# antbern/gridmap-slam-robot

Hardware: AMD Instinct MI355X
Metric: particle-scan evals/sec (higher is better)
Workload: dtype f64; 1 GPU; C3: 16384 particles/GPU x 720 beams (697 hits), 2048x2048 grid @ 0.02 m, full scan step (score+normalise+resample+ray-cast+likelihood rebuild; the rebuild is dirty-tile / factor-table-only: bit-identical results, likelihoodData on demand -- the reference's own every-cell rebuild is cpu_baseline.gpu_like_for_like_ms_per_step); particles_total=16384, particles_per_gpu=16384, beams=720, maps=1, maps_total=1, parallelism=single GPU, inputs=resident in HBM

## Files before the change

### gridmap_slam_robot_amd/csrc/gms_fused_kernels.hip

```cpp
#include "gms_map_kernels.hip"
#include "gms_pf_kernels.hip"
#include "gms_slam_kernels.hip"

#ifndef GMS_APPLY_BLOCKS_RIDING
#define GMS_APPLY_BLOCKS_RIDING 512
#endif

#ifndef RCF_RAYS
#define RCF_RAYS 4
#endif

template <bool LOGNORM>
__global__ void __launch_bounds__(256)
k_norm_raycast(GridDev g, const gms_beam *__restrict__ beams, int32_t B, uint32_t *__restrict__ cnt, int32_t *__restrict__ bbox,
               int32_t nw_max, uint32_t n_ray_blocks,
               const double *__restrict__ partials, int64_t nblk_global, double *__restrict__ w, const float *__restrict__ pose,
               int32_t n, int64_t offset, PackedParticle *__restrict__ packed, double *__restrict__ cum,
               double *__restrict__ chunk_tot, int64_t nchunks, double *__restrict__ p2, PfStatsDev *__restrict__ stats,
               uint32_t n_norm_blocks, double *__restrict__ logd, uint32_t *__restrict__ cnt_pend, const int32_t *__restrict__ bbox_pend,
               uint32_t n_near_blocks, const double *__restrict__ logw_lognorm, uint32_t *__restrict__ res_ticket,
               double *__restrict__ res_pre) {
    extern __shared__ __align__(16) unsigned char smem[];
    GMS_STAMP(GMS_STAMP_ROW(2, blockIdx.x), 0);
    if (blockIdx.x >= n_ray_blocks + n_norm_blocks) {
        apply_body(g, logd, cnt_pend, bbox_pend, nullptr, blockIdx.x - n_ray_blocks - n_norm_blocks, 0,
                   gridDim.x - n_ray_blocks - n_norm_blocks);
        GMS_STAMP(GMS_STAMP_ROW(2, blockIdx.x), 15);
        return;
    }
    if (blockIdx.x < n_ray_blocks) {
        __shared__ RedLds L;
        __shared__ float s_pose[3];
        const int cols[4] = { COL_SUM, COL_XW, COL_YW, COL_TW };
        double f[4];
        if (LOGNORM) {
            fold_lognorm<4>(partials, nblk_global, cols, f, L);
// ... 1 lines not shown
            fold_sums<4>(partials, nblk_global, cols, f, L);
        }
        if (threadIdx.x == 0) {
            s_pose[0] = (float)(f[1] / f[0]);
            s_pose[1] = (float)(f[2] / f[0]);
            s_pose[2] = (float)(f[3] / f[0]);
        }
        __syncthreads();
        GMS_STAMP(GMS_STAMP_ROW(2, blockIdx.x), 1);
        if (blockIdx.x >= n_ray_blocks - n_near_blocks)
            raycast_near_body(g, beams, B, B, nullptr, 0, cnt, bbox, blockIdx.x - (n_ray_blocks - n_near_blocks), 0, smem, s_pose);
        else
            raycast_body<false, RCF_RAYS, 4>(g, beams, B, B, nullptr, 0, nullptr, cnt, bbox, nullptr, nullptr, 0, nullptr, nw_max, blockIdx.x, 0,
                                             smem, s_pose, n_near_blocks ? 1 : 0);
    } else {
        normalize_pack_body(partials, nblk_global, w, pose, n, offset, packed, cum, chunk_tot, nchunks, p2, stats,
                            blockIdx.x - n_ray_blocks, 0, LOGNORM ? logw_lognorm : (const double *)nullptr, res_ticket, n_norm_blocks,
                            res_pre, smem);
        GMS_STAMP(GMS_STAMP_ROW(2, blockIdx.x), 14);
    }
}

__global__ void __launch_bounds__(256)
k_partials_apply(double *__restrict__ w, double *__restrict__ logw, const float *__restrict__ pose, int32_t n, int64_t offset,
                 int64_t nblk_global, double *__restrict__ partials, const double *__restrict__ part, int32_t part_nseg,
                 GridDev g, double *__restrict__ logd, uint32_t *__restrict__ cnt, const int32_t *__restrict__ bbox,
                 int32_t *__restrict__ bbox_idle, PfStatsDev *__restrict__ lognorm_stats) {
    if (blockIdx.x < (uint32_t)nblk_global)
        partials_body(w, logw, pose, n, offset, nblk_global, partials, part, part_nseg, blockIdx.x, blockIdx.y, lognorm_stats);
    else
        apply_body(g, logd, cnt, bbox, bbox_idle, blockIdx.x - (uint32_t)nblk_global, blockIdx.y, gridDim.x - (uint32_t)nblk_global);
}

// ... 78 lines not shown
                double d_center, double d_theta, gms_beam *__restrict__ beams_out, uint32_t n_deskew_blocks,
                float *__restrict__ pose, float *__restrict__ cs, int32_t n, int64_t offset, double d_center_sd, double d_theta_sd,
                uint64_t seed, uint64_t sequence) {
    if (blockIdx.x < n_deskew_blocks)
        deskew_body(angle, distance, hit, length, d_center, d_theta, beams_out, (int32_t)(blockIdx.x * 256u + threadIdx.x));
    else
        motion_body(pose, cs, n, offset, d_center, d_theta, d_center_sd, d_theta_sd, seed, sequence, 0,
                    (int32_t)((blockIdx.x - n_deskew_blocks) * 256u + threadIdx.x));
}

bool gms_can_pair_launches(const gms_pf *pf, int32_t B) {
    const gms_map *m = pf->map;
    return pf->n_maps == 1 && B > 0 && B <= GMS_MAX_BEAMS && !m->need_full_build && m->pair_launches;
}

void gms_launch_norm_raycast(gms_pf *pf, const double *d_partials, PackedParticle *d_packed_local, bool own,
                             const gms_beam *d_beams, int32_t B) {
    gms_map *m = pf->map;
    ProfScope ps(m, GMS_K_RAYCAST);
    const uint32_t n_near = rc_near_blocks(m, B);
    const uint32_t n_ray = (uint32_t)((B + RCF_RAYS - 1) / RCF_RAYS) + n_near, n_norm = (uint32_t)((pf->n + 255) / 256);
    const int64_t nch = nchunks_of(pf);
    const size_t smem_pre = own ? (size_t)(nch + 1 + (nch + 63) / 64 + 1) * sizeof(double) : 0;
    size_t smem = rc_smem(m, RCF_RAYS, n_near);
    if (smem < smem_pre) smem = smem_pre;
    uint32_t n_apply = 0;
    if (m->apply_pending) {
        const int32_t all = ((m->gd.W + APPLY_TW - 1) / APPLY_TW) * ((m->gd.H + APPLY_TH - 1) / APPLY_TH);
        n_apply = (uint32_t)(all < GMS_APPLY_BLOCKS_RIDING ? all : GMS_APPLY_BLOCKS_RIDING);
    }
    int32_t *pend = m->d_bbox + (size_t)m->bbox_cur * 4;
    int32_t *bb = n_apply ? m->d_bbox + (size_t)(1 - m->bbox_cur) * 4 : pend;
    const bool lognorm = gms_pf_lognorm_now(pf);
#define NR_LAUNCH(LN)                                                                                                                 \
    do {                                                                                                                              \
        if (smem > 48 * 1024)                                                                                                         \
            hipFuncSetAttribute(reinterpret_cast<const void *>(&k_norm_raycast<LN>), hipFuncAttributeMaxDynamicSharedMemorySize, (int)smem); \
        hipLaunchKernelGGL(k_norm_raycast<LN>, dim3(n_ray + n_norm + n_apply), dim3(256), smem, m->stream, m->gd, d_beams, B, m->d_cnt, bb, \
                           rc_nw_max(m), n_ray, d_partials, nblk_global_of(pf), pf->d_w, pf->d_pose, pf->n, pf->offset, d_packed_local, \
                           own ? pf->d_cum : (double *)nullptr, own ? pf->d_chunk_tot : (double *)nullptr, nchunks_of(pf),          \
                           own ? pf->d_p2 : (double *)nullptr, pf->d_stats, n_norm, m->d_log, m->d_cnt_pend, pend, n_near,          \
                           LN ? (const double *)pf->d_logw : (const double *)nullptr, own ? pf->d_res_ticket : (uint32_t *)nullptr,       \
                           pf->d_res_pre);                                                                                              \
    } while (0)
    if (lognorm) NR_LAUNCH(true); else NR_LAUNCH(false);
#undef NR_LAUNCH
    if (n_apply) gms_apply_done(m);
    pf_normalized(pf, own, own);
}

void gms_launch_partials_apply(gms_pf *pf, double *d_partials, bool apply_rides_later) {
    gms_map *m = pf->map;
    if (!m->apply_pending || apply_rides_later) { gms_launch_pf_partials(pf, d_partials); return; }
    ProfScope ps(m, GMS_K_REDUCE);
    const int64_t nblk = nblk_global_of(pf);
    const int32_t all = ((m->gd.W + APPLY_TW - 1) / APPLY_TW) * ((m->gd.H + APPLY_TH - 1) / APPLY_TH);
    const uint32_t n_apply = (uint32_t)(all < GMS_APPLY_BLOCKS ? all : GMS_APPLY_BLOCKS);
    int32_t *cur = m->d_bbox + (size_t)m->bbox_cur * m->n_maps * 4, *idle = m->d_bbox + (size_t)(1 - m->bbox_cur) * m->n_maps * 4;
    PfStatsDev *lognorm_stats = gms_pf_lognorm_now(pf) ? pf->d_stats : (PfStatsDev *)nullptr;
    hipLaunchKernelGGL(k_partials_apply, dim3((uint32_t)nblk + n_apply, pf->n_maps), dim3(256), 0, m->stream, pf->d_w, pf->d_logw,
                       pf->d_pose, pf->n, pf->offset, nblk, d_partials,
                       pf->pending_nseg ? (const double *)pf->d_part : (const double *)nullptr, pf->pending_nseg, m->gd, m->d_log,
                       m->d_cnt_pend, cur, idle, lognorm_stats);
    pf_weights_combined(pf);
    gms_apply_done(m);
}

void gms_launch_lik_resample(gms_pf *pf, double fraction) {
// ... 92 lines not shown
```

### gridmap_slam_robot_amd/csrc/gms_host.hip

```cpp
#include <math.h>
#include <dlfcn.h>
#include <stdarg.h>
#include <stddef.h>
#include <stdio.h>
#include <stdlib.h>
#include <string.h>

#include <new>
#include <algorithm>
#include <vector>

#include "gms_internal.h"

static thread_local char g_err[512] = "";

int gms_fail(int code, const char *fmt, ...) {
    va_list ap;
    va_start(ap, fmt);
    vsnprintf(g_err, sizeof(g_err), fmt, ap);
    va_end(ap);
    return code;
}

static int32_t j_d2i_host(double d) {
// ... 1277 lines not shown
    return slam_update_impl(pf, nullptr, &mo, dev_beams, B, B, r01, resample_fraction, integrate);
}

static int slam_update_impl(gms_pf *pf, const float *dev_xytheta, const MotionModel *motion, const gms_beam *dev_beams, int32_t B,
                            int32_t beam_stride, const double *r01, double resample_fraction, int32_t integrate) {
    REQUIRE(pf && dev_beams && r01, "null argument");
    int rc = refuse_owned_maps(pf);
    if (rc) return rc;
    gms_map *m = pf->map;
    if (pf_is_shard(pf))
        return gms_fail(GMS_ERR_STATE, "sharded filter: the collectives belong to the caller (see distributed.py)");
    const ScanIn at_pose = dev_scan(dev_beams, B, beam_stride, nullptr, pf, 0);
    rc = set_poses_and_score_dev(pf, dev_xytheta, dev_beams, B, beam_stride, pf->refine != 0, motion);
    const bool pair = !rc && integrate && !pf->reference_order && beam_stride == B;
    if (pair && gms_can_pair_launches(pf, B)) {
        gms_launch_partials_apply(pf, pf->d_partials, true);
        gms_launch_norm_raycast(pf, pf->d_partials, pf->d_global_own, true, dev_beams, B);
        return paired_likelihood_resample(pf, r01, resample_fraction);
    }
    if (pair && pf->n_maps > 1 && B > 0 && !m->need_full_build && m->pair_launches) {
        const bool ride = gms_raycast_tiled(m, B);
        gms_launch_partials_apply(pf, pf->d_partials, ride);
        gms_launch_pf_apply_partials(pf, pf->d_partials, pf->d_global_own, true);
        ScanDev d;
        scan_pose(m, at_pose, &d);
        gms_launch_raycast(m, dev_beams, B, B, d.poses, d.pose_stride, ride);
        return paired_likelihood_resample(pf, r01, resample_fraction);
    }
    if (!rc) rc = gms_pf_normalize(pf, nullptr);
    if (!rc && resample_fraction >= 0.0) rc = gms_pf_resample_if(pf, r01, resample_fraction);
    if (!rc && integrate) rc = map_scan(m, at_pose, SCAN_UPDATE_MAY_DEFER);
    return rc;
// ... 517 lines not shown
```

### gridmap_slam_robot_amd/csrc/gms_internal.h

```cpp
#pragma once

#include <hip/hip_runtime.h>
#include <stdint.h>

#include <vector>

#include "gridmapslam.h"

struct GridDev {
    int32_t W, H;
    int64_t cells;
    double posx, posy;
    double res;
    double rinv;
    float resf;
    double l_free, l_occ;
    int32_t extra;
    float half_tol;
    double z_hit;
    double c_rand;
    double inv_max;
    int32_t ktaps, khalf;
    int32_t fpitch;
    uint32_t fneutral;
// ... 359 lines not shown
bool gms_set_stamp_buffer(gms_map *m, void *dev_buffer);
void gms_launch_spin(gms_map *m, double us);
void gms_launch_copy(gms_map *m, void *dst, const void *src, size_t nbytes);
void gms_invalidate_tile_state(gms_map *m);
void gms_launch_get_raw(gms_map *m, int32_t mi, int32_t x, int32_t y, double *d_out2);
void gms_launch_debug_f32(gms_map *m, int32_t op, const float *d_a, float *d_out, int64_t n);
int gms_view_check(const gms_view *v, int32_t W, int32_t H, const char *what, int64_t *bytes);
int gms_view_staging(gms_map *m, int64_t image_bytes, unsigned char **base);
void gms_launch_view(gms_map *m, const double *src, const gms_view *v, void *d_out);

void gms_launch_pf_init(gms_pf *pf);
void gms_launch_pf_pose_trig(gms_pf *pf, const float *d_src);
void gms_launch_pf_combine(gms_pf *pf);
void gms_launch_pf_motion(gms_pf *pf, double d_center, double d_theta, uint64_t seed, uint64_t sequence);
void gms_launch_pf_chunk_sums(gms_pf *pf);
void gms_launch_partials_apply(gms_pf *pf, double *d_partials, bool apply_rides_later = false);
bool gms_can_pair_launches(const gms_pf *pf, int32_t B);
void gms_launch_norm_raycast(gms_pf *pf, const double *d_partials, PackedParticle *d_packed_local, bool own,
                             const gms_beam *d_beams, int32_t B);
void gms_launch_lik_resample(gms_pf *pf, double fraction);
void gms_launch_deskew_motion(gms_pf *pf, const double *d_angle, const double *d_distance, const uint8_t *d_hit, int32_t length,
                              double d_center, double d_theta, uint64_t seed, uint64_t sequence);
void gms_launch_partials_pack_apply(gms_pf *pf, bool apply_rides_later = false);
void gms_launch_raycast_norm_chunks(gms_pf *pf, const gms_beam *d_beams, int32_t B, bool raycast);
void gms_launch_pf_fold_neff(gms_pf *pf);
struct MotionModel {
    double d_center, d_theta;
    uint64_t seed, sequence;
};
static inline void motion_deviations(double d_center, double d_theta, double *d_center_sd, double *d_theta_sd) {
    *d_center_sd = (0.01 + fabs(d_center) * 0.05) / 2;
    *d_theta_sd = 5 * (3.141592653589793 / 180.0) + 0.1 * fabs(d_theta);
}
void gms_launch_pf_score(gms_pf *pf, const gms_beam *d_beams, int32_t B, int32_t beam_stride, const float *d_pose_src = nullptr,
                         const MotionModel *motion = nullptr);
void gms_launch_pf_partials(gms_pf *pf, double *d_partials);
bool gms_pf_lognorm_now(const gms_pf *pf);
void gms_launch_pf_pack(gms_pf *pf, PackedParticle *d_packed);
void gms_launch_pf_apply_partials(gms_pf *pf, const double *d_partials, PackedParticle *d_packed_local, bool own);
void gms_launch_pf_stats_only(gms_pf *pf, const double *d_partials, PfStatsDev *d_stats_out);
void gms_launch_pf_resample(gms_pf *pf, double fraction );
void gms_launch_pf_refine(gms_pf *pf, const gms_beam *d_beams, int32_t B, int32_t beam_stride);
void gms_launch_pf_normalize_seq(gms_pf *pf, PfStatsDev *d_stats_out, bool normalise);
void gms_launch_pf_resample_seq(gms_pf *pf, double fraction);
SlamBufs gms_slam_bufs(const gms_slam *s);
void gms_launch_slam_likelihood(gms_map *m, const SlamBufs &sb, int32_t n);
void gms_launch_slam_deskew(gms_map *m, const double *angle, const double *distance, const uint8_t *hit, int32_t L, int32_t S, int32_t Lmax,
                            int32_t length, double d_center, double d_theta, const SlamFilterArgs *tab_src, SlamFilterArgs *tab_dst, gms_beam *d_out,
                            int32_t out_pitch);
void gms_launch_slam_particle(gms_pf *pf, const gms_beam *d_beams, int32_t B, const SlamBufs &sb, bool field_in_memory, const MotionModel *motion,
                              int32_t integrate, int64_t code_words, const SlamBatch *batch = nullptr);
void gms_launch_slam_likelihood_codes(gms_map *m, const SlamBufs &sb, int64_t code_words, int32_t n, int32_t plane);
// ... 33 lines not shown
```

### gridmap_slam_robot_amd/csrc/gms_pf_kernels.hip

```cpp
#include "gms_device.h"

#define SCAN_CHUNK 64
#define RES_SUB_MAX_CHUNKS 1024

__global__ void k_pf_init(float *pose, float *cs, double *w, double *logw, int64_t total, double w0) {
    int64_t i = (int64_t)blockIdx.x * blockDim.x + threadIdx.x;
    if (i < total) {
        pose[3 * i] = 0.0f; pose[3 * i + 1] = 0.0f; pose[3 * i + 2] = 0.0f;
        cs[2 * i] = 1.0f; cs[2 * i + 1] = 0.0f;
        w[i] = w0; logw[i] = 0.0;
    }
}

__global__ void __launch_bounds__(256)
k_pose_trig(const float *__restrict__ src, float *__restrict__ dst, float *__restrict__ cs, int64_t total) {
    const int64_t i = (int64_t)blockIdx.x * blockDim.x + threadIdx.x;
    if (i >= total) return;
    const float x = src[3 * i], y = src[3 * i + 1], th = src[3 * i + 2];
    dst[3 * i] = x; dst[3 * i + 1] = y; dst[3 * i + 2] = th;
    float c, s;
    pose_trig(th, c, s);
    cs[2 * i] = c; cs[2 * i + 1] = s;
}

// ... 384 lines not shown
    double m[GMS_PARTIAL_STRIDE][MAX_WAVES];
};

#define COL_SUM 0
#define COL_MAX 1
#define COL_ARG 2
#define COL_NZ 3
#define COL_MLW 4
#define COL_SQ 5
#define COL_XW 6
#define COL_YW 7
#define COL_TW 8

static_assert(EPT == 1, "the log-normalising form of block_partials takes one particle per thread");
__device__ __forceinline__ double lognorm_ref(double m) { return m > -INFINITY ? m : 0.0; }
__device__ __forceinline__ void block_partials(double *__restrict__ w, double *__restrict__ logw,
                                               const float *__restrict__ pose, int64_t cnt, int64_t base,
                                               double out[GMS_PARTIAL_STRIDE], RedLds &L,
                                               const double *__restrict__ part = nullptr, int32_t part_mi = 0,
                                               int32_t part_n = 0, int32_t part_nseg = 0, int64_t part_p0 = 0,
                                               bool lognorm = false) {
    const int32_t tl = threadIdx.x & (GRP - 1);
    double s = 0.0, nz = 0.0, mv = -INFINITY, mx = 9.0e15, ml = -INFINITY, sq = 0.0, xw = 0.0, yw = 0.0, tw = 0.0;
#pragma unroll
    for (int e0 = 0; e0 < EPT; e0 += EPB) {
        double v[EPB], lw[EPB];
        float px[EPB], py[EPB], pt[EPB];
#pragma unroll
        for (int e = 0; e < EPB; e++) {
            const int64_t i = tl + (e0 + e) * GRP;
            const bool in = i < cnt;
            if (part) {
                v[e] = 0.0; lw[e] = -INFINITY;
                if (in) {
                    combine_segments(part, part_mi, part_n, part_nseg, part_p0 + i, v[e], lw[e]);
                    w[i] = v[e]; logw[i] = lw[e];
                }
            } else {
                v[e] = in ? w[i] : 0.0;
                lw[e] = in ? logw[i] : -INFINITY;
            }
            px[e] = in ? pose[3 * i] : 0.0f; py[e] = in ? pose[3 * i + 1] : 0.0f; pt[e] = in ? pose[3 * i + 2] : 0.0f;
        }
        if (lognorm) {
            double mloc = lw[0] == lw[0] ? lw[0] : -INFINITY;
#define GMS_STEP_(O) { const double v2 = wave_xor<O>(mloc); if (v2 > mloc) mloc = v2; }
            GMS_BUTTERFLY(GMS_STEP_)
#undef GMS_STEP_
            const int32_t wv = threadIdx.x >> 6, g4 = (wv >> 2) << 2;
            __syncthreads();
            if ((threadIdx.x & 63) == 0) L.b[wv] = mloc;
            __syncthreads();
            double mb = L.b[g4];
            for (int k = 1; k < 4; k++) if (L.b[g4 + k] > mb) mb = L.b[g4 + k];
            if (tl < cnt) v[0] = exp(lw[0] - lognorm_ref(mb));
        }
#pragma unroll
        for (int e = 0; e < EPB; e++) {
            const int64_t i = tl + (e0 + e) * GRP;
            if (i < cnt) {
                s += v[e];
                sq += v[e] * v[e];
                xw += (double)px[e] * v[e];
                yw += (double)py[e] * v[e];
                tw += angle_constrain((double)pt[e]) * v[e];
                if (v[e] == 0.0) nz += 1.0;
                const double key = lognorm ? lw[e] : v[e];
                if (key > mv) { mv = key; mx = (double)(base + i); }
                else if (mx > 8.0e15 && key == key) { mv = key; mx = (double)(base + i); }
                if (lw[e] > ml) ml = lw[e];
            }
        }
    }
    GMS_STAMP(GMS_STAMP_ROW(1, blockIdx.x), 2);
    double sums[6] = { s, nz, sq, xw, yw, tw };
#pragma unroll
    for (int c = 0; c < 6; c++) sums[c] = wave_sum_f64(sums[c]);
    double mli = 0.0;
#define GMS_STEP_(O) { const double v2 = wave_xor<O>(mv), i2 = wave_xor<O>(mx); argmax_merge(mv, mx, v2, i2); \
                       const double l2 = wave_xor<O>(ml); if (l2 > ml) ml = l2; }
    GMS_BUTTERFLY(GMS_STEP_)
#undef GMS_STEP_
    const int32_t wave = threadIdx.x >> 6, g4 = (wave >> 2) << 2;
    GMS_STAMP(GMS_STAMP_ROW(1, blockIdx.x), 3);
    __syncthreads();
    if ((threadIdx.x & 63) == 0) {
#pragma unroll
        for (int c = 0; c < 6; c++) L.m[c][wave] = sums[c];
        L.m[6][wave] = mv; L.m[7][wave] = mx; L.m[8][wave] = ml;
    }
    __syncthreads();
    GMS_STAMP(GMS_STAMP_ROW(1, blockIdx.x), 4);
#pragma unroll
    for (int c = 0; c < 6; c++) sums[c] = ((L.m[c][g4] + L.m[c][g4 + 1]) + L.m[c][g4 + 2]) + L.m[c][g4 + 3];
    mv = L.m[6][g4]; mx = L.m[7][g4]; ml = L.m[8][g4];
    for (int k = 1; k < 4; k++) {
        argmax_merge(mv, mx, L.m[6][g4 + k], L.m[7][g4 + k]);
        if (L.m[8][g4 + k] > ml) ml = L.m[8][g4 + k];
    }
    (void)mli;
    out[COL_SUM] = sums[0]; out[COL_NZ] = sums[1]; out[COL_SQ] = sums[2];
    out[COL_XW] = sums[3]; out[COL_YW] = sums[4]; out[COL_TW] = sums[5];
    out[COL_MAX] = mv; out[COL_ARG] = mx; out[COL_MLW] = ml;
}

__device__ __forceinline__ double fold_sum(const double *__restrict__ p, int64_t nblk, int col, double *lds) {
    double acc = 0.0;
    for (int64_t b = threadIdx.x & (GRP - 1); b < nblk; b += GRP) acc += p[b * GMS_PARTIAL_STRIDE + col];
    return group_sum(acc, lds);
}

template <int NC>
__device__ __forceinline__ void fold_sums(const double *__restrict__ p, int64_t nblk, const int (&col)[NC], double (&out)[NC],
                                          RedLds &L) {
    static_assert(NC <= GMS_PARTIAL_STRIDE, "RedLds::m has GMS_PARTIAL_STRIDE rows");
    double acc[NC];
#pragma unroll
// ... 86 lines not shown
    for (int c = 0; c < NC; c++) out[c] = ((L.m[c][g4] + L.m[c][g4 + 1]) + L.m[c][g4 + 2]) + L.m[c][g4 + 3];
    return M;
}

__device__ __forceinline__ void fold_argmax(const double *__restrict__ p, int64_t nblk, int colv, int coli, double &mv,
                                            double &mx, RedLds &L) {
    mv = -INFINITY; mx = 9.0e15;
    bool first = true;
    for (int64_t b = threadIdx.x & (GRP - 1); b < nblk; b += GRP) {
        const double v2 = p[b * GMS_PARTIAL_STRIDE + colv], i2 = coli >= 0 ? p[b * GMS_PARTIAL_STRIDE + coli] : (double)b;
        if (first) { mv = v2; mx = i2; first = false; } else argmax_merge(mv, mx, v2, i2);
    }
    group_argmax(mv, mx, L.a, L.b);
}

__device__ __forceinline__ double fold_stats(const double *__restrict__ p, int64_t nblk, PfStatsDev *s, bool write,
                                             const float *__restrict__ pose, int64_t pose_base, int64_t pose_n, RedLds &L,
                                             const PackedParticle *__restrict__ glob = nullptr, bool lognorm = false, double *ref_out = nullptr) {
    double ml = 0.0, mli;
    if (!write) {
        if (!lognorm) return fold_sum(p, nblk, COL_SUM, L.a);
        const int c1[1] = { COL_SUM };
        double f1[1];
        ml = fold_lognorm<1>(p, nblk, c1, f1, L);
        if (ref_out) *ref_out = ml;
        return f1[0];
    }
    const int cols[5] = { COL_SUM, COL_NZ, COL_XW, COL_YW, COL_TW };
    double f[5];
    if (lognorm) { ml = fold_lognorm<5>(p, nblk, cols, f, L); if (ref_out) *ref_out = ml; }
    else fold_sums<5>(p, nblk, cols, f, L);
    const double sum = f[0], nz = f[1], xw = f[2], yw = f[3], tw = f[4];
    double mv, mx;
    fold_argmax(p, nblk, COL_MAX, COL_ARG, mv, mx, L);
    if (!lognorm) fold_argmax(p, nblk, COL_MLW, -1, ml, mli, L);
    if (threadIdx.x == 0) {
        s->n_ambiguous = 0;
        s->weight_sum = sum;
        s->max_w = lognorm ? exp(ml - lognorm_ref(ml)) : mv;
        s->strongest = mx < 8.0e15 ? (int32_t)mx : 0;
        if (!lognorm) s->n_zero = (int32_t)nz;
// ... 25 lines not shown
    for (int64_t b = threadIdx.x & (GRP - 1); b < nblk; b += GRP) { a += load_coherent<COHERENT>(&p2[2 * b]); q += load_coherent<COHERENT>(&p2[2 * b + 1]); }
    norm_sum = group_sum(a, lds);
    const double qq = group_sum(q, lds);
    sq_sum = qq / (norm_sum * norm_sum);
}

__global__ void __launch_bounds__(256)
k_fold_neff(const double *__restrict__ p2_all, int64_t nblk, PfStatsDev *__restrict__ stats) {
    __shared__ RedLds L;
    const int32_t mi = blockIdx.x;
    double ns, sq;
    fold_neff(p2_all + (size_t)mi * nblk * 2, nblk, ns, sq, L.a);
    if (threadIdx.x == 0) { stats[mi].norm_sum = ns; stats[mi].sq_sum = sq; }
}

__device__ __forceinline__ void
partials_body(double *__restrict__ w, double *__restrict__ logw, const float *__restrict__ pose, int32_t n,
              int64_t offset, int64_t nblk_global, double *__restrict__ partials, const double *__restrict__ part,
              int32_t part_nseg, uint32_t bx, uint32_t by, PfStatsDev *__restrict__ lognorm_stats = nullptr) {
    __shared__ RedLds L;
    const int32_t mi = (int32_t)by;
    if (lognorm_stats && bx == 0 && threadIdx.x == 0) lognorm_stats[mi].n_zero = 0;
    const int64_t gb = bx;
    const int64_t lb = gb - offset / GMS_BLOCK;
    const int64_t nlb = ((int64_t)n + GMS_BLOCK - 1) / GMS_BLOCK;
    double *p = partials + ((size_t)mi * nblk_global + gb) * GMS_PARTIAL_STRIDE;
    if (lb < 0 || lb >= nlb) {
        if (threadIdx.x < GMS_PARTIAL_STRIDE) p[threadIdx.x] = 0.0;
        return;
    }
    double out[GMS_PARTIAL_STRIDE];
    const size_t o = (size_t)mi * n + lb * GMS_BLOCK;
    block_partials(w + o, logw + o, pose + 3 * o, block_count(n, lb), offset + lb * GMS_BLOCK, out, L, part, mi, n,
                   part_nseg, lb * GMS_BLOCK, lognorm_stats != nullptr);
    if (threadIdx.x == 0)
        for (int k = 0; k < GMS_PARTIAL_STRIDE; k++) p[k] = out[k];
}

__global__ void __launch_bounds__(256)
k_partials(double *__restrict__ w, double *__restrict__ logw, const float *__restrict__ pose, int32_t n,
           int64_t offset, int64_t nblk_global, double *__restrict__ partials, const double *__restrict__ part,
           int32_t part_nseg, PfStatsDev *__restrict__ lognorm_stats) {
    GMS_STAMP(GMS_STAMP_ROW(1, blockIdx.x), 0);
    partials_body(w, logw, pose, n, offset, nblk_global, partials, part, part_nseg, blockIdx.x, blockIdx.y, lognorm_stats);
    GMS_STAMP(GMS_STAMP_ROW(1, blockIdx.x), 1);
}

__device__ __forceinline__ double *chunk_sub_of(double *chunk_tot_all, int64_t nchunks, int32_t n_maps, int32_t mi) {
    return chunk_tot_all + (size_t)n_maps * (nchunks + 1) + (size_t)mi * nchunks * 8;
}
__device__ __forceinline__ void block_chunk_scan(double v, int64_t i, int64_t n_pop, int64_t blk, int64_t nchunks,
                                                 double *__restrict__ cum, double *__restrict__ chunk_tot,
                                                 double *__restrict__ p2_blk, double *__restrict__ sub, bool through = false) {
    __shared__ double s_ct[4][2];
    const int32_t lane = threadIdx.x & 63, wave = threadIdx.x >> 6;
    double inc = v;
#pragma unroll
    for (int o = 1; o < 64; o <<= 1) {
        const double up = __shfl_up(inc, o, GMS_WAVE);
// ... 48 lines not shown
                const double up = __shfl_up(inc, o, GMS_WAVE);
                if (lane >= o) inc += up;
            }
            const double excl = __shfl_up(inc, 1, GMS_WAVE);
            if (sidx < nsuper) sup[sidx] = s0 == 0 ? (lane == 0 ? 0.0 : excl) : carry + (lane == 0 ? 0.0 : excl);
            const double tot = __shfl(inc, 63, GMS_WAVE);
            carry = s0 == 0 ? tot : carry + tot;
        }
        if (lane == 0) off[nchunks] = carry;
    }
    __syncthreads();
    for (int64_t c = 64 + threadIdx.x; c < nchunks; c += blockDim.x) off[c] = sup[c >> 6] + off[c];
    __syncthreads();
}

__device__ __forceinline__ void
resample_prefix_last(const double *__restrict__ p2, int64_t nblk, const double *__restrict__ tot, int64_t nchunks, uint32_t *__restrict__ ticket,
                     uint32_t n_blocks, double *__restrict__ pre, PfStatsDev *__restrict__ stats, unsigned char *smem, double *lds) {
    __shared__ int32_t s_last;
    asm volatile("s_waitcnt vmcnt(0)" ::: "memory");
    __syncthreads();
    if (threadIdx.x == 0) {
        const uint32_t t = __hip_atomic_fetch_add(ticket, 1u, __ATOMIC_RELAXED, __HIP_MEMORY_SCOPE_AGENT);
        s_last = t == n_blocks - 1;
        if (s_last) __hip_atomic_store(ticket, 0u, __ATOMIC_RELAXED, __HIP_MEMORY_SCOPE_AGENT);
    }
    __syncthreads();
    if (!s_last) return;
    double *off = reinterpret_cast<double *>(smem);
    double tv[8];
#pragma unroll
    for (int k = 0; k < 8; k++) { const int64_t c = (int64_t)threadIdx.x + k * (int64_t)blockDim.x; tv[k] = c < nchunks ? load_coherent<true>(&tot[c]) : 0.0; }
    double norm_sum, sq_sum;
// ... 1 lines not shown
#pragma unroll
    for (int k = 0; k < 8; k++) { const int64_t c = (int64_t)threadIdx.x + k * (int64_t)blockDim.x; if (c < nchunks) off[c] = tv[k]; }
    for (int64_t c0 = (int64_t)threadIdx.x + 8 * (int64_t)blockDim.x; c0 < nchunks; c0 += 8 * (int64_t)blockDim.x) {
        double v[8];
#pragma unroll
        for (int k = 0; k < 8; k++) { const int64_t c = c0 + k * (int64_t)blockDim.x; v[k] = c < nchunks ? load_coherent<true>(&tot[c]) : 0.0; }
#pragma unroll
        for (int k = 0; k < 8; k++) { const int64_t c = c0 + k * (int64_t)blockDim.x; if (c < nchunks) off[c] = v[k]; }
    }
    chunk_offsets_scan(off, nchunks);
    for (int64_t c = threadIdx.x; c <= nchunks; c += blockDim.x) pre[c] = off[c];
    if (threadIdx.x == 0) {
        pre[nchunks + 1] = norm_sum; pre[nchunks + 2] = sq_sum;
        stats->norm_sum = norm_sum; stats->sq_sum = sq_sum;
    }
    GMS_STAMP(GMS_STAMP_ROW(2, blockIdx.x), 13);
}

__device__ __forceinline__ void
normalize_pack_body(const double *__restrict__ partials_all, int64_t nblk_global, double *__restrict__ w,
                    const float *__restrict__ pose, int32_t n, int64_t offset, PackedParticle *__restrict__ packed,
                    double *__restrict__ cum, double *__restrict__ chunk_tot, int64_t nchunks,
                    double *__restrict__ p2_all, PfStatsDev *__restrict__ stats, uint32_t bx, uint32_t by,
                    const double *__restrict__ logw_lognorm = nullptr, uint32_t *__restrict__ ticket = nullptr,
                    uint32_t n_blocks = 0, double *__restrict__ pre = nullptr, unsigned char *smem = nullptr) {
    __shared__ RedLds L;
    const int32_t mi = (int32_t)by;
    const double *p = partials_all + (size_t)mi * nblk_global * GMS_PARTIAL_STRIDE;
    double M = 0.0;
    const double sum = fold_stats(p, nblk_global, stats + mi, bx == 0, pose + (size_t)mi * n * 3, offset, n, L, nullptr, logw_lognorm != nullptr, &M);
    const int32_t i = (int32_t)bx * 256 + threadIdx.x;
    double wn = 0.0;
    if (logw_lognorm) {
        const double v = i < n ? exp(logw_lognorm[(size_t)mi * n + i] - lognorm_ref(M)) : 1.0;
        const int32_t zeros = __popcll(__ballot(v == 0.0));
        if ((threadIdx.x & 63) == 0 && zeros) atomicAdd(&stats[mi].n_zero, zeros);
        if (i < n) w[(size_t)mi * n + i] = v;
    }
    if (i < n) {
        const size_t gi = (size_t)mi * n + i;
        wn = w[gi] / sum;
        w[gi] = wn;
        PackedParticle pp;
        pp.w = wn; pp.x = pose[3 * gi]; pp.y = pose[3 * gi + 1]; pp.theta = pose[3 * gi + 2]; pp.pad = 0u;
        packed[gi] = pp;
    }
    if (cum)
        block_chunk_scan(wn, i, n, bx, nchunks, cum + (size_t)mi * n, chunk_tot + (size_t)mi * (nchunks + 1),
                         p2_all + ((size_t)mi * nblk_global + bx) * 2, chunk_sub_of(chunk_tot, nchunks, (int32_t)gridDim.y, mi),
                         ticket != nullptr);
    if (cum && ticket) resample_prefix_last(p2_all + (size_t)mi * nblk_global * 2, nblk_global, chunk_tot + (size_t)mi * (nchunks + 1),
                                            nchunks, ticket + mi, n_blocks, pre + (size_t)mi * (nchunks + 3), stats + mi, smem, L.a);
}

__global__ void __launch_bounds__(256)
k_normalize_pack(const double *__restrict__ partials_all, int64_t nblk_global, double *__restrict__ w,
                 const float *__restrict__ pose, int32_t n, int64_t offset, PackedParticle *__restrict__ packed,
                 double *__restrict__ cum, double *__restrict__ chunk_tot, int64_t nchunks,
                 double *__restrict__ p2_all, PfStatsDev *__restrict__ stats, const double *__restrict__ logw_lognorm) {
    normalize_pack_body(partials_all, nblk_global, w, pose, n, offset, packed, cum, chunk_tot, nchunks, p2_all, stats, blockIdx.x,
                        blockIdx.y, logw_lognorm);
}

__device__ __forceinline__ void
chunk_sums_body(const PackedParticle *__restrict__ glob_all, int64_t n_global, int64_t nchunks, double *__restrict__ cum_all,
                double *__restrict__ chunk_tot, double *__restrict__ p2_all, int64_t nblk_global, PfStatsDev *__restrict__ stats,
                uint32_t bx, uint32_t by) {
// ... 515 lines not shown
    if (motion) { std::swap(pf->d_pose, pf->d_pose2); std::swap(pf->d_cs, pf->d_cs2); }
    pf_scored(pf, nseg);
}

void gms_launch_pf_combine(gms_pf *pf) {
    if (!pf->pending_nseg) return;
    gms_map *m = pf->map;
    ProfScope ps(m, GMS_K_SCORE);
    hipLaunchKernelGGL(k_score_combine, dim3((pf->n + 255) / 256, pf->n_maps), dim3(256), 0, m->stream, pf->d_part, pf->n,
                       pf->pending_nseg, pf->d_w, pf->d_logw);
    pf_weights_combined(pf);
}

bool gms_pf_lognorm_now(const gms_pf *pf) { return pf->log_norm && pf->score_fresh; }

void gms_launch_pf_partials(gms_pf *pf, double *d_partials) {
    gms_map *m = pf->map;
    ProfScope ps(m, GMS_K_REDUCE);
    const int64_t nblk = nblk_global_of(pf);
    hipLaunchKernelGGL(k_partials, dim3((unsigned)nblk, pf->n_maps), dim3(256), 0, m->stream, pf->d_w, pf->d_logw,
                       pf->d_pose, pf->n, pf->offset, nblk, d_partials,
                       pf->pending_nseg ? (const double *)pf->d_part : (const double *)nullptr, pf->pending_nseg,
                       gms_pf_lognorm_now(pf) ? pf->d_stats : (PfStatsDev *)nullptr);
    pf_weights_combined(pf);
}

void gms_launch_pf_apply_partials(gms_pf *pf, const double *d_partials, PackedParticle *d_packed_local, bool own) {
    gms_map *m = pf->map;
    ProfScope ps(m, GMS_K_REDUCE);
    const int64_t nblk = nblk_global_of(pf);
    hipLaunchKernelGGL(k_normalize_pack, dim3((pf->n + 255) / 256, pf->n_maps), dim3(256), 0, m->stream, d_partials, nblk,
                       pf->d_w, pf->d_pose, pf->n, pf->offset, d_packed_local, own ? pf->d_cum : (double *)nullptr,
                       own ? pf->d_chunk_tot : (double *)nullptr, nchunks_of(pf), own ? pf->d_p2 : (double *)nullptr, pf->d_stats,
                       gms_pf_lognorm_now(pf) ? (const double *)pf->d_logw : (const double *)nullptr);
    pf_normalized(pf, own, false);
}

void gms_launch_pf_stats_only(gms_pf *pf, const double *d_partials, PfStatsDev *d_stats_out) {
// ... 73 lines not shown
```

Baseline: 371.0 million particle-scan evals/s.

## Defer argmax/zero/max-logw stats from partials kernel into normalise-pack pass

```diff
diff --git a/gridmap_slam_robot_amd/csrc/gms_fused_kernels.hip b/gridmap_slam_robot_amd/csrc/gms_fused_kernels.hip
--- a/gridmap_slam_robot_amd/csrc/gms_fused_kernels.hip
+++ b/gridmap_slam_robot_amd/csrc/gms_fused_kernels.hip
@@ -10,7 +10,7 @@
 #define RCF_RAYS 4
 #endif
 
-template <bool LOGNORM>
+template <bool LOGNORM, bool DEFER>
 __global__ void __launch_bounds__(256)
 k_norm_raycast(GridDev g, const gms_beam *__restrict__ beams, int32_t B, uint32_t *__restrict__ cnt, int32_t *__restrict__ bbox,
                int32_t nw_max, uint32_t n_ray_blocks,
@@ -18,8 +18,9 @@
                int32_t n, int64_t offset, PackedParticle *__restrict__ packed, double *__restrict__ cum,
                double *__restrict__ chunk_tot, int64_t nchunks, double *__restrict__ p2, PfStatsDev *__restrict__ stats,
                uint32_t n_norm_blocks, double *__restrict__ logd, uint32_t *__restrict__ cnt_pend, const int32_t *__restrict__ bbox_pend,
-               uint32_t n_near_blocks, const double *__restrict__ logw_lognorm, uint32_t *__restrict__ res_ticket,
-               double *__restrict__ res_pre) {
+               uint32_t n_near_blocks, const double *__restrict__ logw, uint32_t *__restrict__ res_ticket,
+               double *__restrict__ res_pre, double *partials_rw) {
+    static_assert(!(LOGNORM && DEFER), "the block-relative partial vector needs every column in front of this launch");
     extern __shared__ __align__(16) unsigned char smem[];
     GMS_STAMP(GMS_STAMP_ROW(2, blockIdx.x), 0);
     if (blockIdx.x >= n_ray_blocks + n_norm_blocks) {
@@ -51,9 +52,9 @@
             raycast_body<false, RCF_RAYS, 4>(g, beams, B, B, nullptr, 0, nullptr, cnt, bbox, nullptr, nullptr, 0, nullptr, nw_max, blockIdx.x, 0,
                                              smem, s_pose, n_near_blocks ? 1 : 0);
     } else {
-        normalize_pack_body(partials, nblk_global, w, pose, n, offset, packed, cum, chunk_tot, nchunks, p2, stats,
-                            blockIdx.x - n_ray_blocks, 0, LOGNORM ? logw_lognorm : (const double *)nullptr, res_ticket, n_norm_blocks,
-                            res_pre, smem);
+        normalize_pack_body<DEFER>(partials, nblk_global, w, pose, n, offset, packed, cum, chunk_tot, nchunks, p2, stats,
+                                   blockIdx.x - n_ray_blocks, 0, LOGNORM ? logw : (const double *)nullptr, res_ticket, n_norm_blocks,
+                                   res_pre, smem, partials_rw, logw);
         GMS_STAMP(GMS_STAMP_ROW(2, blockIdx.x), 14);
     }
 }
@@ -162,8 +163,8 @@
     return pf->n_maps == 1 && B > 0 && B <= GMS_MAX_BEAMS && !m->need_full_build && m->pair_launches;
 }
 
-void gms_launch_norm_raycast(gms_pf *pf, const double *d_partials, PackedParticle *d_packed_local, bool own,
-                             const gms_beam *d_beams, int32_t B) {
+void gms_launch_norm_raycast(gms_pf *pf, double *d_partials, PackedParticle *d_packed_local, bool own,
+                             const gms_beam *d_beams, int32_t B, bool deferred) {
     gms_map *m = pf->map;
     ProfScope ps(m, GMS_K_RAYCAST);
     const uint32_t n_near = rc_near_blocks(m, B);
@@ -180,26 +181,26 @@
     int32_t *pend = m->d_bbox + (size_t)m->bbox_cur * 4;
     int32_t *bb = n_apply ? m->d_bbox + (size_t)(1 - m->bbox_cur) * 4 : pend;
     const bool lognorm = gms_pf_lognorm_now(pf);
-#define NR_LAUNCH(LN)                                                                                                                 \
+#define NR_LAUNCH(LN, DF)                                                                                                                 \
     do {                                                                                                                              \
         if (smem > 48 * 1024)                                                                                                         \
-            hipFuncSetAttribute(reinterpret_cast<const void *>(&k_norm_raycast<LN>), hipFuncAttributeMaxDynamicSharedMemorySize, (int)smem); \
-        hipLaunchKernelGGL(k_norm_raycast<LN>, dim3(n_ray + n_norm + n_apply), dim3(256), smem, m->stream, m->gd, d_beams, B, m->d_cnt, bb, \
+            hipFuncSetAttribute(reinterpret_cast<const void *>(&k_norm_raycast<LN, DF>), hipFuncAttributeMaxDynamicSharedMemorySize, (int)smem); \
+        hipLaunchKernelGGL((k_norm_raycast<LN, DF>), dim3(n_ray + n_norm + n_apply), dim3(256), smem, m->stream, m->gd, d_beams, B, m->d_cnt, bb, \
                            rc_nw_max(m), n_ray, d_partials, nblk_global_of(pf), pf->d_w, pf->d_pose, pf->n, pf->offset, d_packed_local, \
                            own ? pf->d_cum : (double *)nullptr, own ? pf->d_chunk_tot : (double *)nullptr, nchunks_of(pf),          \
                            own ? pf->d_p2 : (double *)nullptr, pf->d_stats, n_norm, m->d_log, m->d_cnt_pend, pend, n_near,          \
-                           LN ? (const double *)pf->d_logw : (const double *)nullptr, own ? pf->d_res_ticket : (uint32_t *)nullptr,       \
-                           pf->d_res_pre);                                                                                              \
+                           (LN || DF) ? (const double *)pf->d_logw : (const double *)nullptr, own ? pf->d_res_ticket : (uint32_t *)nullptr,  \
+                           pf->d_res_pre, DF ? d_partials : (double *)nullptr);                                                         \
     } while (0)
-    if (lognorm) NR_LAUNCH(true); else NR_LAUNCH(false);
+    if (lognorm) NR_LAUNCH(true, false); else if (deferred && own) NR_LAUNCH(false, true); else NR_LAUNCH(false, false);
 #undef NR_LAUNCH
     if (n_apply) gms_apply_done(m);
     pf_normalized(pf, own, own);
 }
 
-void gms_launch_partials_apply(gms_pf *pf, double *d_partials, bool apply_rides_later) {
-    gms_map *m = pf->map;
-    if (!m->apply_pending || apply_rides_later) { gms_launch_pf_partials(pf, d_partials); return; }
+void gms_launch_partials_apply(gms_pf *pf, double *d_partials, bool apply_rides_later, bool trimmed) {
+    gms_map *m = pf->map;
+    if (!m->apply_pending || apply_rides_later) { gms_launch_pf_partials(pf, d_partials, trimmed); return; }
     ProfScope ps(m, GMS_K_REDUCE);
     const int64_t nblk = nblk_global_of(pf);
     const int32_t all = ((m->gd.W + APPLY_TW - 1) / APPLY_TW) * ((m->gd.H + APPLY_TH - 1) / APPLY_TH);
diff --git a/gridmap_slam_robot_amd/csrc/gms_host.hip b/gridmap_slam_robot_amd/csrc/gms_host.hip
--- a/gridmap_slam_robot_amd/csrc/gms_host.hip
+++ b/gridmap_slam_robot_amd/csrc/gms_host.hip
@@ -1315,8 +1315,9 @@
     rc = set_poses_and_score_dev(pf, dev_xytheta, dev_beams, B, beam_stride, pf->refine != 0, motion);
     const bool pair = !rc && integrate && !pf->reference_order && beam_stride == B;
     if (pair && gms_can_pair_launches(pf, B)) {
-        gms_launch_partials_apply(pf, pf->d_partials, true);
-        gms_launch_norm_raycast(pf, pf->d_partials, pf->d_global_own, true, dev_beams, B);
+        const bool trimmed = gms_pf_trimmed_step(pf);
+        gms_launch_partials_apply(pf, pf->d_partials, true, trimmed);
+        gms_launch_norm_raycast(pf, pf->d_partials, pf->d_global_own, true, dev_beams, B, trimmed);
         return paired_likelihood_resample(pf, r01, resample_fraction);
     }
     if (pair && pf->n_maps > 1 && B > 0 && !m->need_full_build && m->pair_launches) {
diff --git a/gridmap_slam_robot_amd/csrc/gms_internal.h b/gridmap_slam_robot_amd/csrc/gms_internal.h
--- a/gridmap_slam_robot_amd/csrc/gms_internal.h
+++ b/gridmap_slam_robot_amd/csrc/gms_internal.h
@@ -397,10 +397,10 @@
 void gms_launch_pf_combine(gms_pf *pf);
 void gms_launch_pf_motion(gms_pf *pf, double d_center, double d_theta, uint64_t seed, uint64_t sequence);
 void gms_launch_pf_chunk_sums(gms_pf *pf);
-void gms_launch_partials_apply(gms_pf *pf, double *d_partials, bool apply_rides_later = false);
+void gms_launch_partials_apply(gms_pf *pf, double *d_partials, bool apply_rides_later = false, bool trimmed = false);
 bool gms_can_pair_launches(const gms_pf *pf, int32_t B);
-void gms_launch_norm_raycast(gms_pf *pf, const double *d_partials, PackedParticle *d_packed_local, bool own,
-                             const gms_beam *d_beams, int32_t B);
+void gms_launch_norm_raycast(gms_pf *pf, double *d_partials, PackedParticle *d_packed_local, bool own,
+                             const gms_beam *d_beams, int32_t B, bool deferred = false);
 void gms_launch_lik_resample(gms_pf *pf, double fraction);
 void gms_launch_deskew_motion(gms_pf *pf, const double *d_angle, const double *d_distance, const uint8_t *d_hit, int32_t length,
                               double d_center, double d_theta, uint64_t seed, uint64_t sequence);
@@ -417,8 +417,9 @@
 }
 void gms_launch_pf_score(gms_pf *pf, const gms_beam *d_beams, int32_t B, int32_t beam_stride, const float *d_pose_src = nullptr,
                          const MotionModel *motion = nullptr);
-void gms_launch_pf_partials(gms_pf *pf, double *d_partials);
+void gms_launch_pf_partials(gms_pf *pf, double *d_partials, bool trimmed = false);
 bool gms_pf_lognorm_now(const gms_pf *pf);
+bool gms_pf_trimmed_step(const gms_pf *pf);
 void gms_launch_pf_pack(gms_pf *pf, PackedParticle *d_packed);
 void gms_launch_pf_apply_partials(gms_pf *pf, const double *d_partials, PackedParticle *d_packed_local, bool own);
 void gms_launch_pf_stats_only(gms_pf *pf, const double *d_partials, PfStatsDev *d_stats_out);
diff --git a/gridmap_slam_robot_amd/csrc/gms_pf_kernels.hip b/gridmap_slam_robot_amd/csrc/gms_pf_kernels.hip
--- a/gridmap_slam_robot_amd/csrc/gms_pf_kernels.hip
+++ b/gridmap_slam_robot_amd/csrc/gms_pf_kernels.hip
@@ -422,6 +422,7 @@
 
 static_assert(EPT == 1, "the log-normalising form of block_partials takes one particle per thread");
 __device__ __forceinline__ double lognorm_ref(double m) { return m > -INFINITY ? m : 0.0; }
+template <bool SUMS4 = false>
 __device__ __forceinline__ void block_partials(double *__restrict__ w, double *__restrict__ logw,
                                                const float *__restrict__ pose, int64_t cnt, int64_t base,
                                                double out[GMS_PARTIAL_STRIDE], RedLds &L,
@@ -429,7 +430,7 @@
                                                int32_t part_n = 0, int32_t part_nseg = 0, int64_t part_p0 = 0,
                                                bool lognorm = false) {
     const int32_t tl = threadIdx.x & (GRP - 1);
-    double s = 0.0, nz = 0.0, mv = -INFINITY, mx = 9.0e15, ml = -INFINITY, sq = 0.0, xw = 0.0, yw = 0.0, tw = 0.0;
+    double s = 0.0, nz = 0.0, mv = -INFINITY, mx = 9.0e15, ml = -INFINITY, xw = 0.0, yw = 0.0, tw = 0.0;
 #pragma unroll
     for (int e0 = 0; e0 < EPT; e0 += EPB) {
         double v[EPB], lw[EPB];
@@ -446,11 +447,11 @@
                 }
             } else {
                 v[e] = in ? w[i] : 0.0;
-                lw[e] = in ? logw[i] : -INFINITY;
+                lw[e] = !SUMS4 && in ? logw[i] : -INFINITY;
             }
             px[e] = in ? pose[3 * i] : 0.0f; py[e] = in ? pose[3 * i + 1] : 0.0f; pt[e] = in ? pose[3 * i + 2] : 0.0f;
         }
-        if (lognorm) {
+        if (!SUMS4 && lognorm) {
             double mloc = lw[0] == lw[0] ? lw[0] : -INFINITY;
 #define GMS_STEP_(O) { const double v2 = wave_xor<O>(mloc); if (v2 > mloc) mloc = v2; }
             GMS_BUTTERFLY(GMS_STEP_)
@@ -468,47 +469,64 @@
             const int64_t i = tl + (e0 + e) * GRP;
             if (i < cnt) {
                 s += v[e];
-                sq += v[e] * v[e];
                 xw += (double)px[e] * v[e];
                 yw += (double)py[e] * v[e];
                 tw += angle_constrain((double)pt[e]) * v[e];
-                if (v[e] == 0.0) nz += 1.0;
-                const double key = lognorm ? lw[e] : v[e];
-                if (key > mv) { mv = key; mx = (double)(base + i); }
-                else if (mx > 8.0e15 && key == key) { mv = key; mx = (double)(base + i); }
-                if (lw[e] > ml) ml = lw[e];
+                if (!SUMS4) {
+                    if (v[e] == 0.0) nz += 1.0;
+                    const double key = lognorm ? lw[e] : v[e];
+                    if (key > mv) { mv = key; mx = (double)(base + i); }
+                    else if (mx > 8.0e15 && key == key) { mv = key; mx = (double)(base + i); }
+                    if (lw[e] > ml) ml = lw[e];
+                }
             }
         }
     }
     GMS_STAMP(GMS_STAMP_ROW(1, blockIdx.x), 2);
-    double sums[6] = { s, nz, sq, xw, yw, tw };
-#pragma unroll
-    for (int c = 0; c < 6; c++) sums[c] = wave_sum_f64(sums[c]);
-    double mli = 0.0;
+    const int32_t wave = threadIdx.x >> 6, g4 = (wave >> 2) << 2;
+    if (SUMS4) {
+        double sums[4] = { s, xw, yw, tw };
+#pragma unroll
+        for (int c = 0; c < 4; c++) sums[c] = wave_sum_f64(sums[c]);
+        GMS_STAMP(GMS_STAMP_ROW(1, blockIdx.x), 3);
+        __syncthreads();
+        if ((threadIdx.x & 63) == 0) {
+#pragma unroll
+            for (int c = 0; c < 4; c++) L.m[c][wave] = sums[c];
+        }
+        __syncthreads();
+        GMS_STAMP(GMS_STAMP_ROW(1, blockIdx.x), 4);
+#pragma unroll
+        for (int c = 0; c < 4; c++) sums[c] = ((L.m[c][g4] + L.m[c][g4 + 1]) + L.m[c][g4 + 2]) + L.m[c][g4 + 3];
+        out[COL_SUM] = sums[0]; out[COL_XW] = sums[1]; out[COL_YW] = sums[2]; out[COL_TW] = sums[3];
+        out[COL_SQ] = 0.0;
+        return;
+    }
+    double sums[5] = { s, nz, xw, yw, tw };
+#pragma unroll
+    for (int c = 0; c < 5; c++) sums[c] = wave_sum_f64(sums[c]);
 #define GMS_STEP_(O) { const double v2 = wave_xor<O>(mv), i2 = wave_xor<O>(mx); argmax_merge(mv, mx, v2, i2); \
                        const double l2 = wave_xor<O>(ml); if (l2 > ml) ml = l2; }
     GMS_BUTTERFLY(GMS_STEP_)
 #undef GMS_STEP_
-    const int32_t wave = threadIdx.x >> 6, g4 = (wave >> 2) << 2;
     GMS_STAMP(GMS_STAMP_ROW(1, blockIdx.x), 3);
     __syncthreads();
     if ((threadIdx.x & 63) == 0) {
 #pragma unroll
-        for (int c = 0; c < 6; c++) L.m[c][wave] = sums[c];
+        for (int c = 0; c < 5; c++) L.m[c][wave] = sums[c];
         L.m[6][wave] = mv; L.m[7][wave] = mx; L.m[8][wave] = ml;
     }
     __syncthreads();
     GMS_STAMP(GMS_STAMP_ROW(1, blockIdx.x), 4);
 #pragma unroll
-    for (int c = 0; c < 6; c++) sums[c] = ((L.m[c][g4] + L.m[c][g4 + 1]) + L.m[c][g4 + 2]) + L.m[c][g4 + 3];
+    for (int c = 0; c < 5; c++) sums[c] = ((L.m[c][g4] + L.m[c][g4 + 1]) + L.m[c][g4 + 2]) + L.m[c][g4 + 3];
     mv = L.m[6][g4]; mx = L.m[7][g4]; ml = L.m[8][g4];
     for (int k = 1; k < 4; k++) {
         argmax_merge(mv, mx, L.m[6][g4 + k], L.m[7][g4 + k]);
         if (L.m[8][g4 + k] > ml) ml = L.m[8][g4 + k];
     }
-    (void)mli;
-    out[COL_SUM] = sums[0]; out[COL_NZ] = sums[1]; out[COL_SQ] = sums[2];
-    out[COL_XW] = sums[3]; out[COL_YW] = sums[4]; out[COL_TW] = sums[5];
+    out[COL_SUM] = sums[0]; out[COL_NZ] = sums[1]; out[COL_SQ] = 0.0;
+    out[COL_XW] = sums[2]; out[COL_YW] = sums[3]; out[COL_TW] = sums[4];
     out[COL_MAX] = mv; out[COL_ARG] = mx; out[COL_MLW] = ml;
 }
 
@@ -625,6 +643,7 @@
     group_argmax(mv, mx, L.a, L.b);
 }
 
+template <bool SUMS_ONLY = false>
 __device__ __forceinline__ double fold_stats(const double *__restrict__ p, int64_t nblk, PfStatsDev *s, bool write,
                                              const float *__restrict__ pose, int64_t pose_base, int64_t pose_n, RedLds &L,
                                              const PackedParticle *__restrict__ glob = nullptr, bool lognorm = false, double *ref_out = nullptr) {
@@ -636,6 +655,20 @@
         ml = fold_lognorm<1>(p, nblk, c1, f1, L);
         if (ref_out) *ref_out = ml;
         return f1[0];
+    }
+    if (SUMS_ONLY) {
+        const int cols4[4] = { COL_SUM, COL_XW, COL_YW, COL_TW };
+        double f4[4];
+        fold_sums<4>(p, nblk, cols4, f4, L);
+        if (threadIdx.x == 0) {
+            s->n_ambiguous = 0;
+            s->weight_sum = f4[0];
+            s->xs = f4[1]; s->ys = f4[2]; s->ts = f4[3];
+            s->wpose[0] = (float)(f4[1] / f4[0]);
+            s->wpose[1] = (float)(f4[2] / f4[0]);
+            s->wpose[2] = (float)(f4[3] / f4[0]);
+        }
+        return f4[0];
     }
     const int cols[5] = { COL_SUM, COL_NZ, COL_XW, COL_YW, COL_TW };
     double f[5];
@@ -691,6 +724,7 @@
     if (threadIdx.x == 0) { stats[mi].norm_sum = ns; stats[mi].sq_sum = sq; }
 }
 
+template <bool SUMS4 = false>
 __device__ __forceinline__ void
 partials_body(double *__restrict__ w, double *__restrict__ logw, const float *__restrict__ pose, int32_t n,
               int64_t offset, int64_t nblk_global, double *__restrict__ partials, const double *__restrict__ part,
@@ -708,18 +742,24 @@
     }
     double out[GMS_PARTIAL_STRIDE];
     const size_t o = (size_t)mi * n + lb * GMS_BLOCK;
-    block_partials(w + o, logw + o, pose + 3 * o, block_count(n, lb), offset + lb * GMS_BLOCK, out, L, part, mi, n,
-                   part_nseg, lb * GMS_BLOCK, lognorm_stats != nullptr);
-    if (threadIdx.x == 0)
-        for (int k = 0; k < GMS_PARTIAL_STRIDE; k++) p[k] = out[k];
-}
-
+    block_partials<SUMS4>(w + o, logw + o, pose + 3 * o, block_count(n, lb), offset + lb * GMS_BLOCK, out, L, part, mi, n,
+                          part_nseg, lb * GMS_BLOCK, lognorm_stats != nullptr);
+    if (threadIdx.x == 0) {
+        if (SUMS4) {
+            p[COL_SUM] = out[COL_SUM]; p[COL_SQ] = out[COL_SQ]; p[COL_XW] = out[COL_XW]; p[COL_YW] = out[COL_YW]; p[COL_TW] = out[COL_TW];
+        } else {
+            for (int k = 0; k < GMS_PARTIAL_STRIDE; k++) p[k] = out[k];
+        }
+    }
+}
+
+template <bool SUMS4>
 __global__ void __launch_bounds__(256)
 k_partials(double *__restrict__ w, double *__restrict__ logw, const float *__restrict__ pose, int32_t n,
            int64_t offset, int64_t nblk_global, double *__restrict__ partials, const double *__restrict__ part,
            int32_t part_nseg, PfStatsDev *__restrict__ lognorm_stats) {
     GMS_STAMP(GMS_STAMP_ROW(1, blockIdx.x), 0);
-    partials_body(w, logw, pose, n, offset, nblk_global, partials, part, part_nseg, blockIdx.x, blockIdx.y, lognorm_stats);
+    partials_body<SUMS4>(w, logw, pose, n, offset, nblk_global, partials, part, part_nseg, blockIdx.x, blockIdx.y, lognorm_stats);
     GMS_STAMP(GMS_STAMP_ROW(1, blockIdx.x), 1);
 }
 
@@ -798,9 +838,12 @@
     __syncthreads();
 }
 
+template <bool STATS>
 __device__ __forceinline__ void
 resample_prefix_last(const double *__restrict__ p2, int64_t nblk, const double *__restrict__ tot, int64_t nchunks, uint32_t *__restrict__ ticket,
-                     uint32_t n_blocks, double *__restrict__ pre, PfStatsDev *__restrict__ stats, unsigned char *smem, double *lds) {
+                     uint32_t n_blocks, double *__restrict__ pre, PfStatsDev *__restrict__ stats, unsigned char *smem, RedLds &L,
+                     const double *partials = nullptr, const float *__restrict__ pose = nullptr, int64_t pose_base = 0, int64_t pose_n = 0) {
+    double *lds = L.a;
     __shared__ int32_t s_last;
     asm volatile("s_waitcnt vmcnt(0)" ::: "memory");
     __syncthreads();
@@ -832,21 +875,58 @@
         pre[nchunks + 1] = norm_sum; pre[nchunks + 2] = sq_sum;
         stats->norm_sum = norm_sum; stats->sq_sum = sq_sum;
     }
+    if (STATS) {
+        double nz = 0.0, mv = -INFINITY, mx = 9.0e15, ml = -INFINITY;
+        bool first = true;
+        for (int64_t b = threadIdx.x & (GRP - 1); b < nblk; b += GRP) {
+            double v[4];
+#pragma unroll
+            for (int k = 0; k < 4; k++) v[k] = load_coherent<true>(&partials[b * GMS_PARTIAL_STRIDE + COL_MAX + k]);
+            if (first) { mv = v[0]; mx = v[1]; first = false; } else argmax_merge(mv, mx, v[0], v[1]);
+            nz += v[2];
+            if (v[3] > ml) ml = v[3];
+        }
+        nz = wave_sum_f64(nz);
+#define GMS_STEP_(O) { const double v2 = wave_xor<O>(mv), i2 = wave_xor<O>(mx); argmax_merge(mv, mx, v2, i2); \
+                       const double l2 = wave_xor<O>(ml); if (l2 > ml) ml = l2; }
+        GMS_BUTTERFLY(GMS_STEP_)
+#undef GMS_STEP_
+        const int32_t wave = threadIdx.x >> 6, g4 = (wave >> 2) << 2;
+        __syncthreads();
+        if ((threadIdx.x & 63) == 0) { L.m[0][wave] = nz; L.m[1][wave] = mv; L.m[2][wave] = mx; L.m[3][wave] = ml; }
+        __syncthreads();
+        if (threadIdx.x == 0) {
+            nz = ((L.m[0][g4] + L.m[0][g4 + 1]) + L.m[0][g4 + 2]) + L.m[0][g4 + 3];
+            mv = L.m[1][g4]; mx = L.m[2][g4]; ml = L.m[3][g4];
+            for (int k = 1; k < 4; k++) {
+                argmax_merge(mv, mx, L.m[1][g4 + k], L.m[2][g4 + k]);
+                if (L.m[3][g4 + k] > ml) ml = L.m[3][g4 + k];
+            }
+            stats->max_w = mv;
+            stats->strongest = mx < 8.0e15 ? (int32_t)mx : 0;
+            stats->n_zero = (int32_t)nz;
+            stats->max_logw = ml;
+            const int64_t st = (int64_t)stats->strongest - pose_base;
+            if (st >= 0 && st < pose_n) { stats->spose[0] = pose[3 * st]; stats->spose[1] = pose[3 * st + 1]; stats->spose[2] = pose[3 * st + 2]; }
+        }
+    }
     GMS_STAMP(GMS_STAMP_ROW(2, blockIdx.x), 13);
 }
 
+template <bool DEFER = false>
 __device__ __forceinline__ void
 normalize_pack_body(const double *__restrict__ partials_all, int64_t nblk_global, double *__restrict__ w,
                     const float *__restrict__ pose, int32_t n, int64_t offset, PackedParticle *__restrict__ packed,
                     double *__restrict__ cum, double *__restrict__ chunk_tot, int64_t nchunks,
                     double *__restrict__ p2_all, PfStatsDev *__restrict__ stats, uint32_t bx, uint32_t by,
                     const double *__restrict__ logw_lognorm = nullptr, uint32_t *__restrict__ ticket = nullptr,
-                    uint32_t n_blocks = 0, double *__restrict__ pre = nullptr, unsigned char *smem = nullptr) {
+                    uint32_t n_blocks = 0, double *__restrict__ pre = nullptr, unsigned char *smem = nullptr,
+                    double *partials_rw = nullptr, const double *__restrict__ logw = nullptr) {
     __shared__ RedLds L;
     const int32_t mi = (int32_t)by;
     const double *p = partials_all + (size_t)mi * nblk_global * GMS_PARTIAL_STRIDE;
     double M = 0.0;
-    const double sum = fold_stats(p, nblk_global, stats + mi, bx == 0, pose + (size_t)mi * n * 3, offset, n, L, nullptr, logw_lognorm != nullptr, &M);
+    const double sum = fold_stats<DEFER>(p, nblk_global, stats + mi, bx == 0, pose + (size_t)mi * n * 3, offset, n, L, nullptr, logw_lognorm != nullptr, &M);
     const int32_t i = (int32_t)bx * 256 + threadIdx.x;
     double wn = 0.0;
     if (logw_lognorm) {
@@ -855,20 +935,50 @@
         if ((threadIdx.x & 63) == 0 && zeros) atomicAdd(&stats[mi].n_zero, zeros);
         if (i < n) w[(size_t)mi * n + i] = v;
     }
+    double raw = 0.0, lw = -INFINITY;
     if (i < n) {
         const size_t gi = (size_t)mi * n + i;
-        wn = w[gi] / sum;
+        raw = w[gi];
+        if (DEFER) lw = logw[gi];
+        wn = raw / sum;
         w[gi] = wn;
         PackedParticle pp;
         pp.w = wn; pp.x = pose[3 * gi]; pp.y = pose[3 * gi + 1]; pp.theta = pose[3 * gi + 2]; pp.pad = 0u;
         packed[gi] = pp;
     }
+    if (DEFER) {
+        const bool valid = i < n && raw == raw;
+        double mv = valid ? raw : -INFINITY, ml = lw > -INFINITY ? lw : -INFINITY;
+#define GMS_STEP_(O) { const double v2 = wave_xor<O>(mv); if (v2 > mv) mv = v2; const double l2 = wave_xor<O>(ml); if (l2 > ml) ml = l2; }
+        GMS_BUTTERFLY(GMS_STEP_)
+#undef GMS_STEP_
+        const uint64_t at = __ballot(valid && raw == mv);
+        const double mx = at ? (double)(offset + (int64_t)(i - (int32_t)(threadIdx.x & 63)) + (int64_t)__builtin_ctzll(at)) : 9.0e15;
+        const double nz = (double)__popcll(__ballot(i < n && raw == 0.0));
+        const int32_t wave = threadIdx.x >> 6;
+        __syncthreads();
+        if ((threadIdx.x & 63) == 0) { L.m[0][wave] = mv; L.m[1][wave] = mx; L.m[2][wave] = nz; L.m[3][wave] = ml; }
+        __syncthreads();
+        if (threadIdx.x == 0) {
+            double bv = L.m[0][0], bi = L.m[1][0], bz = L.m[2][0], bl = L.m[3][0];
+            for (int k = 1; k < 4; k++) {
+                argmax_merge(bv, bi, L.m[0][k], L.m[1][k]);
+                bz += L.m[2][k];
+                if (L.m[3][k] > bl) bl = L.m[3][k];
+            }
+            double *row = partials_rw + ((size_t)mi * nblk_global + (size_t)(offset / GMS_BLOCK) + bx) * GMS_PARTIAL_STRIDE;
+            store_through(&row[COL_MAX], bv); store_through(&row[COL_ARG], bi); store_through(&row[COL_NZ], bz); store_through(&row[COL_MLW], bl);
+        }
+        GMS_STAMP(GMS_STAMP_ROW(2, blockIdx.x), 6);
+    }
     if (cum)
         block_chunk_scan(wn, i, n, bx, nchunks, cum + (size_t)mi * n, chunk_tot + (size_t)mi * (nchunks + 1),
                          p2_all + ((size_t)mi * nblk_global + bx) * 2, chunk_sub_of(chunk_tot, nchunks, (int32_t)gridDim.y, mi),
                          ticket != nullptr);
-    if (cum && ticket) resample_prefix_last(p2_all + (size_t)mi * nblk_global * 2, nblk_global, chunk_tot + (size_t)mi * (nchunks + 1),
-                                            nchunks, ticket + mi, n_blocks, pre + (size_t)mi * (nchunks + 3), stats + mi, smem, L.a);
+    if (cum && ticket) resample_prefix_last<DEFER>(p2_all + (size_t)mi * nblk_global * 2, nblk_global, chunk_tot + (size_t)mi * (nchunks + 1),
+                                                   nchunks, ticket + mi, n_blocks, pre + (size_t)mi * (nchunks + 3), stats + mi, smem, L,
+                                                   DEFER ? partials_rw + (size_t)mi * nblk_global * GMS_PARTIAL_STRIDE : (const double *)nullptr,
+                                                   pose + (size_t)mi * n * 3, offset, n);
 }
 
 __global__ void __launch_bounds__(256)
@@ -1414,14 +1524,20 @@
 
 bool gms_pf_lognorm_now(const gms_pf *pf) { return pf->log_norm && pf->score_fresh; }
 
-void gms_launch_pf_partials(gms_pf *pf, double *d_partials) {
+bool gms_pf_trimmed_step(const gms_pf *pf) { return pf->n_maps == 1 && !pf_is_shard(pf) && !gms_pf_lognorm_now(pf); }
+
+void gms_launch_pf_partials(gms_pf *pf, double *d_partials, bool trimmed) {
     gms_map *m = pf->map;
     ProfScope ps(m, GMS_K_REDUCE);
     const int64_t nblk = nblk_global_of(pf);
-    hipLaunchKernelGGL(k_partials, dim3((unsigned)nblk, pf->n_maps), dim3(256), 0, m->stream, pf->d_w, pf->d_logw,
-                       pf->d_pose, pf->n, pf->offset, nblk, d_partials,
-                       pf->pending_nseg ? (const double *)pf->d_part : (const double *)nullptr, pf->pending_nseg,
-                       gms_pf_lognorm_now(pf) ? pf->d_stats : (PfStatsDev *)nullptr);
+    const double *part = pf->pending_nseg ? (const double *)pf->d_part : (const double *)nullptr;
+    if (trimmed)
+        hipLaunchKernelGGL(k_partials<true>, dim3((unsigned)nblk, 1), dim3(256), 0, m->stream, pf->d_w, pf->d_logw, pf->d_pose, pf->n,
+                           pf->offset, nblk, d_partials, part, pf->pending_nseg, (PfStatsDev *)nullptr);
+    else
+        hipLaunchKernelGGL(k_partials<false>, dim3((unsigned)nblk, pf->n_maps), dim3(256), 0, m->stream, pf->d_w, pf->d_logw,
+                           pf->d_pose, pf->n, pf->offset, nblk, d_partials, part, pf->pending_nseg,
+                           gms_pf_lognorm_now(pf) ? pf->d_stats : (PfStatsDev *)nullptr);
     pf_weights_combined(pf);
 }
 
```

Measured after the change: 386.6 million particle-scan evals/s (median of 6 runs). 1.04x the previous value.
